# jzhou316/meta-gcn

Measured on AMD Instinct MI355X. Metric: edges/sec GCN fwd+bwd, 10M-edge synth graph F=128, at 1/2/4/8 MI355X, higher is better.
Workload: dtype f32; 1 GPU; config2: Erdos-Renyi N=1M, E=10M (+1M self-loops), F=128, 3-layer GCN (sm, add, bias, ReLU) fwd+bwd; nodes=1000000, edges=10000000, nnz=11000000, feat=128, layers=3, global_batch=1, parallelism=single

## Files before the change

meta-gcn_amd/csrc/fused.hip:

```cpp

#include <string>

#include "mgcn_internal.h"
#include "x6.h"

#ifndef MGCN_NT_AUX
#define MGCN_NT_AUX 2
#endif
#ifndef MGCN_NT_OUT
#define MGCN_NT_OUT 2
#endif

namespace mgcn {
namespace {

using namespace x6;

constexpr int kXwF = 128;
constexpr int kXwRows = 32;
constexpr int kXwWaves = 8;
constexpr int kXwThreads = 64 * kXwWaves;
constexpr int kXwImg = kXwRows * 256;
constexpr int kXwStageLd = kXwF + 8;
constexpr int kXwStage = kXwRows * kXwStageLd * 4;
// ... 292 lines not shown
        mcb = col[mb.beg + my];
        if (w != nullptr) mwb = w[mb.beg + my];
        if constexpr (MAXM) msb = slot_map[mb.beg + my];
      }
    }
    const int64_t ra = da - e0, rb = db - e0;
    const int na = ra <= 0 ? 0 : (ra < 32 ? (int)ra : 32);
    const int nb = rb <= 0 ? 0 : (rb < 32 ? (int)rb : 32);
    const int64_t remw = dm - e0;
    const int nbmax = remw < 32 ? (int)remw : 32;
    for (int k0 = 0; k0 < nbmax; k0 += U) {
      float4 xa[U], xb[U];
      float wa[U], wb[U];
      uint32_t ba[U], bb[U];
#pragma unroll
      for (int u = 0; u < U; ++u) {
        const int k = k0 + u;
        const int ca = bcast_g(mca, grp, k & 31);
        const int cb = bcast_g(mcb, grp, k & 31);
        wa[u] = bcast_g(mwa, grp, k & 31);
        wb[u] = bcast_g(mwb, grp, k & 31);
        const uint32_t oa = k < na ? (uint32_t)ca * ldx_b + 16u * gl : 0xfffffff0u;
        const uint32_t ob = k < nb ? (uint32_t)cb * ldx_b + 16u * gl : 0xfffffff0u;
        xa[u] = __builtin_bit_cast(float4, __builtin_amdgcn_raw_buffer_load_b128(rx, oa, 0, 0));
        xb[u] = __builtin_bit_cast(float4, __builtin_amdgcn_raw_buffer_load_b128(rx, ob, 0, 0));
        if constexpr (MAXM) {
          const int sa = bcast_g(msa, grp, k & 31);
          const int sb = bcast_g(msb, grp, k & 31);
          ba[u] = win[k < na ? (int64_t)sa * 4 + (gl >> 3) : 0];
          bb[u] = win[k < nb ? (int64_t)sb * 4 + (gl >> 3) : 0];
        }
      }
#pragma unroll
      for (int u = 0; u < U; ++u) {
        if constexpr (MAXM) {
          const uint32_t qa = ba[u] >> (4 * (gl & 7)), qb = bb[u] >> (4 * (gl & 7));
          xa[u].x = (qa & 1u) ? xa[u].x : 0.0f;
          xa[u].y = (qa & 2u) ? xa[u].y : 0.0f;
          xa[u].z = (qa & 4u) ? xa[u].z : 0.0f;
          xa[u].w = (qa & 8u) ? xa[u].w : 0.0f;
          xb[u].x = (qb & 1u) ? xb[u].x : 0.0f;
          xb[u].y = (qb & 2u) ? xb[u].y : 0.0f;
          xb[u].z = (qb & 4u) ? xb[u].z : 0.0f;
          xb[u].w = (qb & 8u) ? xb[u].w : 0.0f;
        }
        if (k0 + u < na) {
          aa[0] = __fadd_rn(aa[0], __fmul_rn(xa[u].x, wa[u]));
          aa[1] = __fadd_rn(aa[1], __fmul_rn(xa[u].y, wa[u]));
          aa[2] = __fadd_rn(aa[2], __fmul_rn(xa[u].z, wa[u]));
          aa[3] = __fadd_rn(aa[3], __fmul_rn(xa[u].w, wa[u]));
        }
        if (k0 + u < nb) {
          ab[0] = __fadd_rn(ab[0], __fmul_rn(xb[u].x, wb[u]));
          ab[1] = __fadd_rn(ab[1], __fmul_rn(xb[u].y, wb[u]));
          ab[2] = __fadd_rn(ab[2], __fmul_rn(xb[u].z, wb[u]));
          ab[3] = __fadd_rn(ab[3], __fmul_rn(xb[u].w, wb[u]));
        }
      }
    }
  }
}

struct RowSeq {
  int64_t base;
  int64_t step;
  int64_t n_rows;
  __device__ __forceinline__ int64_t row(int64_t k) const { return base + (k >> 1) * step + 16 * (k & 1); }
};

__device__ __forceinline__ int64_t my_chunks(int64_t n_chunks) {
  return blockIdx.x < n_chunks ? (n_chunks - 1 - blockIdx.x) / gridDim.x + 1 : 0;
}

#if MGCN_EXPERIMENT
constexpr int kTailMaxWg = 1024;
__device__ unsigned long long g_tail[2][kTailMaxWg][4];
#define XTAIL_ENTRY(k)                                           \
  if (threadIdx.x == 0 && blockIdx.x < kTailMaxWg) g_tail[k][blockIdx.x][0] = wall_clock64();
#define XTAIL_EXIT(k, chunks)                                                         \
  if ((threadIdx.x & 63) == 0 && blockIdx.x < kTailMaxWg) {                           \
    atomicMax(&g_tail[k][blockIdx.x][1], (unsigned long long)wall_clock64());         \
    if (threadIdx.x == 0) g_tail[k][blockIdx.x][2] = (unsigned long long)(chunks);    \
  }
#else
#define XTAIL_ENTRY(k)
#define XTAIL_EXIT(k, chunks)
#endif

__device__ __forceinline__ void store_row_terms(char *img_base, int lr, int gl, const float (&v)[4]) {
  uint32_t hi[2], mid[2], lo[2];
  split3_pair(f32x2{v[0], v[1]}, hi[0], mid[0], lo[0]);
  split3_pair(f32x2{v[2], v[3]}, hi[1], mid[1], lo[1]);
  char *img = img_base + img_off(lr, gl >> 1) + 8 * (gl & 1);
  *reinterpret_cast<uint2 *>(img) = make_uint2(hi[0], hi[1]);
  *reinterpret_cast<uint2 *>(img + kXwImg) = make_uint2(mid[0], mid[1]);
  *reinterpret_cast<uint2 *>(img + 2 * kXwImg) = make_uint2(lo[0], lo[1]);
}

__device__ __forceinline__ void mfma_rows(const char *img, const bf16x8 (&b)[3], int ks, int l16,
                                          int g4, f32x4_t (&acc)[2]) {
#pragma unroll
  for (int t = 0; t < 2; ++t) {
    const int off = img_off(16 * t + l16, 4 * ks + g4);
    const bf16x8 ah = *reinterpret_cast<const bf16x8 *>(img + off);
    const bf16x8 am = *reinterpret_cast<const bf16x8 *>(img + kXwImg + off);
    const bf16x8 al = *reinterpret_cast<const bf16x8 *>(img + 2 * kXwImg + off);
    acc[t] = mfma16_x6(ah, am, al, b[0], b[1], b[2], acc[t]);
  }
}

constexpr int kXfBuf = 3 * kXwImg;
constexpr int kXfStageOff = 2 * kXfBuf;
constexpr int kXfLds = kXfStageOff + 2 * kXfStage;
static_assert(2 * kXfLds <= 160 * 1024, "two forward workgroups per CU");

struct XwArgs {
  int64_t n_rows;
  const int64_t *rowptr;
  const int32_t *col;
  const float *w;
  const float *X;
  int64_t ldx;
  int64_t n_cols;
  const float *W;
  int64_t ldw;
  const float *bias;
  float *Y;
  int64_t ldy;
  uint32_t *relu_mask;
  float *Z;
  int64_t ldz;
  int mean;
  int relu;
  int32_t dyn_first;
  uint32_t *claim;
  int32_t *mail;
  const uint32_t *pk;
  uint32_t pk_bytes, pk_rbits, pk_head;
  uint32_t pk_base[64];
};

template <int U, bool PK = false, bool DYN = false>
__global__ __launch_bounds__(kXwThreads, 2 * kXwPerCU) void spmm_xw_fwd_kernel(const XwArgs a) {
  static_assert(!(DYN && PK), "the dynamic claim serves the dense forward");
  __shared__ __attribute__((aligned(16))) char lds[kXfLds];
  const int tid = threadIdx.x;
  const int lane = tid & 63;
  const int wave = __builtin_amdgcn_readfirstlane(tid >> 6);
  const int gl = lane & 31, grp = lane >> 5;
  const int l16 = lane & 15, g4 = lane >> 4;
  const int64_t n_chunks = (a.n_rows + kXwRows - 1) / kXwRows;
  const bool has_b = a.bias != nullptr;
  const auto rx = buf_rsrc(PK ? nullptr : a.X, PK ? 0u : (uint32_t)(a.n_cols * a.ldx * 4));
  const uint32_t ldx_b = (uint32_t)a.ldx * 4u;
  Pk128 pk{};
  u32x2 hh[PK ? U : 1];
  if constexpr (PK) {
    pk.r = buf_rsrc(a.pk, a.pk_bytes);
    pk.rbits = a.pk_rbits;
    pk.head = a.pk_head;
    pk.base = a.pk_base[lane];
  }

  const int ncol = 16 * wave + l16;
  bf16x8 wb[4][3];
  {
    const float *wp = a.W + (int64_t)(8 * g4) * a.ldw + ncol;
#pragma unroll
    for (int ks = 0; ks < 4; ++ks) {
// ... 481 lines not shown
  if (g_xw_dyn_rounds <= 0 || g_xw_unroll != 5 || workspace == nullptr ||
      reinterpret_cast<uintptr_t>(workspace) % 4 != 0 || workspace_bytes < xw_dyn_workspace_bytes() || rounds < g_xw_dyn_rounds + 8 ||
      n_chunks >= (int64_t(1) << 30))
    return false;
  a.dyn_first = (int32_t)((rounds - g_xw_dyn_rounds) * grid);
  a.claim = static_cast<uint32_t *>(workspace);
  a.mail = reinterpret_cast<int32_t *>(static_cast<char *>(workspace) + kXwDynMailOff);
  if (hipMemsetAsync(a.claim, 0, sizeof(uint32_t), s) != hipSuccess) {
    *rc = check_launch("hipMemsetAsync");
    return true;
  }
  hipLaunchKernelGGL((spmm_xw_fwd_kernel<5, false, true>), dim3((unsigned)grid), dim3(kXwThreads),
                     0, s, a);
  *rc = check_launch("spmm_xw_fwd_kernel");
  return true;
}

template <int U, bool DX, int EPI, bool MAXM, bool DW = true, bool PK = false>
int launch_xb(const XbArgs &a, int grid, hipStream_t s) {
  hipLaunchKernelGGL((spmm_xw_bwd_kernel<U, DX, EPI, MAXM, DW, PK>), dim3((unsigned)grid),
                     dim3(kXwThreads), 0, s, a);
  return check_launch("spmm_xw_bwd_kernel");
}

template <int U, bool PK = false>
int launch_xb_dx(const XbArgs &a, int epi, int grid, hipStream_t s) {
  if (epi == EPI_RELU_DIV) return launch_xb<U, true, EPI_RELU_DIV, false, false, PK>(a, grid, s);
  if (epi == EPI_RELU) return launch_xb<U, true, EPI_RELU, false, false, PK>(a, grid, s);
  return launch_xb<U, true, EPI_STORE, false, false, PK>(a, grid, s);
}

template <int U, bool MAXM>
int launch_xb_m(const XbArgs &a, int epi, int grid, hipStream_t s) {
  if (a.dX == nullptr) return launch_xb<U, false, EPI_STORE, MAXM>(a, grid, s);
  if (epi == EPI_RELU_DIV) return launch_xb<U, true, EPI_RELU_DIV, MAXM>(a, grid, s);
  if (epi == EPI_RELU) return launch_xb<U, true, EPI_RELU, MAXM>(a, grid, s);
  return launch_xb<U, true, EPI_STORE, MAXM>(a, grid, s);
}

template <int U>
int launch_xb_u(const XbArgs &a, int epi, int grid, hipStream_t s) {
  return a.win_mask != nullptr ? launch_xb_m<U, true>(a, epi, grid, s)
                               : launch_xb_m<U, false>(a, epi, grid, s);
}

constexpr int kBsDws = 2, kBsDwsH = 3, kBsDwsM = 4;
#ifndef MGCN_DS_MASK_RING
#define MGCN_DS_MASK_RING 1
#endif
constexpr int kBsImgSet = 3 * kXwImg;
constexpr int kDsXLd = kXwF + 4;
constexpr int kDsXOff = kBsImgSet;
constexpr int kDsMaskOff = kDsXOff + kXwRows * kDsXLd * 4;
constexpr int kDsDivOff = kDsMaskOff + kXwRows * 16;
constexpr int kDsRingBuf = kDsDivOff + kXwRows * 4;
constexpr int kDsWOff = 2 * kDsRingBuf;
constexpr int kDsCtrOff = kDsWOff + kXwF * kDsXLd * 4;
constexpr int kDsLds = kDsCtrOff + 64;
static_assert(kDsLds <= 160 * 1024, "one DWS workgroup per CU");
static_assert(16 * kXwF * 4 <= kDsWOff, "column-sum fold fits in the ring");
constexpr int kBsNG = 8, kBsNM = 8;
constexpr int kBsThreads = 64 * (kBsNG + kBsNM);

__device__ __forceinline__ int bs_lds_load(const int *p) {
  return __builtin_amdgcn_readfirstlane(
      __hip_atomic_load(p, __ATOMIC_RELAXED, __HIP_MEMORY_SCOPE_WORKGROUP));
}

__device__ __forceinline__ bool bs_wait_ge(const int *p, int target, int *abort_word,
                                           uint32_t limit) {
  for (uint32_t n = 0;; ++n) {
    if (bs_lds_load(p) >= target) break;
    if (bs_lds_load(abort_word) != 0) return false;
    if (n >= limit) {
      __hip_atomic_store(abort_word, 1, __ATOMIC_RELAXED, __HIP_MEMORY_SCOPE_WORKGROUP);
      return false;
    }
    __builtin_amdgcn_s_sleep(1);
  }
  asm volatile("" ::: "memory");
  return true;
}

__device__ __forceinline__ int bs_signal(int *p, int v, int lane) {
  asm volatile("s_waitcnt lgkmcnt(0)" ::: "memory");
  int old = 0;
  if (lane == 0) old = __hip_atomic_fetch_add(p, v, __ATOMIC_RELAXED, __HIP_MEMORY_SCOPE_WORKGROUP);
  return __builtin_amdgcn_readfirstlane(old);
}

__device__ __forceinline__ f32x4_t mfma16_x6_at(const bf16x8 (&w)[3], const bf16x8 &xh,
                                               const bf16x8 &xm, const bf16x8 &xl, f32x4_t c) {
  c = __builtin_amdgcn_mfma_f32_16x16x32_bf16(w[0], xl, c, 0, 0, 0);
  c = __builtin_amdgcn_mfma_f32_16x16x32_bf16(w[2], xh, c, 0, 0, 0);
  c = __builtin_amdgcn_mfma_f32_16x16x32_bf16(w[1], xm, c, 0, 0, 0);
  c = __builtin_amdgcn_mfma_f32_16x16x32_bf16(w[0], xm, c, 0, 0, 0);
  c = __builtin_amdgcn_mfma_f32_16x16x32_bf16(w[1], xh, c, 0, 0, 0);
  return __builtin_amdgcn_mfma_f32_16x16x32_bf16(w[0], xh, c, 0, 0, 0);
}

struct XbsArgs {
  XbArgs b;
  float *hcs_partial;
  int dbg;
  uint32_t spin;
  unsigned *err;
};

template <int U, int EPI, int MODE>
__global__ __launch_bounds__(kBsThreads) void spmm_xw_bwd_ws_kernel(const XbsArgs A) {
  constexpr bool HCS = MODE == kBsDwsH;
  constexpr bool MAXM = MODE == kBsDwsM;
  constexpr bool MRING = MGCN_DS_MASK_RING;
  constexpr int kRing = kDsRingBuf;
  constexpr int kDbgMask = MAXM ? ~0 : mgcn::kDbgMask;
  const XbArgs &a = A.b;
  __shared__ __attribute__((aligned(16))) char lds[kDsLds];
  const int tid = threadIdx.x;
  const int lane = tid & 63;
  const int wave = __builtin_amdgcn_readfirstlane(tid >> 6);
  const int gl = lane & 31, grp = lane >> 5;
  const int l16 = lane & 15, g4 = lane >> 4;
  int *ctr = reinterpret_cast<int *>(lds + kDsCtrOff);
  int *filled = ctr, *mdone = ctr + 2, *freed = ctr + 4, *abort_word = ctr + 8;
  if (tid < 16) ctr[tid] = 0;
#pragma unroll
  for (int j = 0; j < 4; ++j) {
    const int e = tid + kBsThreads * j;
    const float4 v = *reinterpret_cast<const float4 *>(a.W + (int64_t)(e >> 5) * a.ldw + 4 * (e & 31));
    *reinterpret_cast<float4 *>(lds + kDsWOff + 4 * ((e >> 5) * kDsXLd + 4 * (e & 31))) = v;
  }
  __syncthreads();

  const int64_t n_chunks = (a.n_rows + kXwRows - 1) / kXwRows;
  const int64_t n_my = my_chunks(n_chunks);
  auto chunk_of = [&](int64_t i) { return (int64_t)blockIdx.x + i * gridDim.x; };
  XTAIL_ENTRY(1);
  auto rows_in = [&](int64_t c) -> uint32_t {
    const int64_t r = a.n_rows - c * kXwRows;
    return (uint32_t)(r <= 0 ? 0 : r >= kXwRows ? kXwRows : r);
  };

  float cs[4] = {0.0f, 0.0f, 0.0f, 0.0f};
  float hc[4] = {0.0f, 0.0f, 0.0f, 0.0f};
  f32x16 accw[2];
#pragma unroll
  for (int s = 0; s < 2; ++s)
#pragma unroll
    for (int r = 0; r < 16; ++r) accw[s][r] = 0.0f;

  if (wave < kBsNG) {
    const int64_t n_quads = 8 * n_my;
    auto row_of = [&](int64_t k, int second) -> int64_t {
      const int64_t q = wave + kBsNG * k;
      return chunk_of(q >> 3) * kXwRows + 4 * (q & 7) + 2 * second + grp;
    };
    const auto rdy = buf_rsrc(a.dY, (uint32_t)(a.n_cols * a.lddy * 4));
    const uint32_t ldy_b = (uint32_t)a.lddy * 4u;
    RowMeta cur[2] = {}, nxt[2] = {};
#pragma unroll
    for (int j = 0; j < 2; ++j) {
      meta_rowptr(a.rowptr, row_of(0, j), row_of(0, j) < a.n_rows && wave < n_quads, cur[j]);
      if constexpr (MAXM)
        meta_first_m(a.col, a.w, a.slot_map, gl, cur[j]);
      else
        meta_first(a.col, a.w, gl, cur[j]);
      meta_rowptr(a.rowptr, row_of(1, j), row_of(1, j) < a.n_rows && wave + kBsNG < n_quads,
                  nxt[j]);
    }
    int64_t k = 0;
    for (int64_t q = wave; q < n_quads; q += kBsNG, ++k) {
      RowMeta nn[2];
#pragma unroll
      for (int j = 0; j < 2; ++j) {
        if constexpr (MAXM)
          meta_first_m(a.col, a.w, a.slot_map, gl, nxt[j]);
        else
          meta_first(a.col, a.w, gl, nxt[j]);
        const int64_t r2 = row_of(k + 2, j);
        meta_rowptr(a.rowptr, r2, r2 < a.n_rows && q + 2 * kBsNG < n_quads, nn[j]);
      }
      const int64_t i = q >> 3;
      const int64_t c = chunk_of(i);
      const int64_t r0 = c * kXwRows;
      const int lr0 = 4 * (int)(q & 7) + grp;
      u32x4 zv[2] = {};
      if (!(A.dbg & kDbgMask & 4)) {
        const auto rz = buf_rsrc(a.X + r0 * a.ldx, rows_in(c) * (uint32_t)a.ldx * 4u);
#pragma unroll
        for (int j = 0; j < 2; ++j)
          zv[j] = __builtin_amdgcn_raw_buffer_load_b128(
              rz, 4 * (int)((lr0 + 2 * j) * a.ldx + 4 * gl), 0, MGCN_NT_AUX);
      }
      uint32_t mv[2] = {0u, 0u};
      if constexpr (MRING && EPI != EPI_STORE) {
        const auto rm = buf_rsrc(a.relu_mask + r0 * 4, rows_in(c) * 16u);
#pragma unroll
        for (int j = 0; j < 2; ++j)
          if (gl < 4) mv[j] = __builtin_amdgcn_raw_buffer_load_b32(rm, 4 * ((lr0 + 2 * j) * 4 + gl), 0, 0);
        if constexpr (EPI == EPI_RELU_DIV) {
          const auto rd = buf_rsrc(a.row_div + r0, rows_in(c) * 4u);
#pragma unroll
          for (int j = 0; j < 2; ++j)
            if (gl == 4) mv[j] = __builtin_amdgcn_raw_buffer_load_b32(rd, 4 * (lr0 + 2 * j), 0, 0);
        }
      }
      u32x4 yv[2] = {};
      if constexpr (HCS) {
        const auto ry = buf_rsrc(a.dY + r0 * a.lddy, rows_in(c) * (uint32_t)a.lddy * 4u);
#pragma unroll
        for (int j = 0; j < 2; ++j)
          yv[j] = __builtin_amdgcn_raw_buffer_load_b128(
              ry, 4 * (int)((lr0 + 2 * j) * a.lddy + 4 * gl), 0, 0);
      }
      float acc[2][4];
      gather_row2_meta<U, MAXM>(rdy, ldy_b, a.col, a.w, cur[0], cur[1], gl, grp, acc[0], acc[1],
                                a.win_mask, a.slot_map);
      if constexpr (HCS) {
#pragma unroll
        for (int j = 0; j < 2; ++j) {
          const float4 y = __builtin_bit_cast(float4, yv[j]);
          hc[0] = __fadd_rn(hc[0], y.x);
          hc[1] = __fadd_rn(hc[1], y.y);
          hc[2] = __fadd_rn(hc[2], y.z);
          hc[3] = __fadd_rn(hc[3], y.w);
        }
      }
#pragma unroll
      for (int j = 0; j < 2; ++j) {
        const int64_t row = r0 + lr0 + 2 * j;
        if (a.row_scale != nullptr && row < a.n_rows) {
          const float sc = a.row_scale[row];
#pragma unroll
          for (int t = 0; t < 4; ++t) acc[j][t] = __fmul_rn(acc[j][t], sc);
        }
      }
      const int b = (int)(i & 1);
      const int gen = (int)(i >> 1);
      if (!bs_wait_ge(freed + b, gen, abort_word, A.spin)) break;
      char *buf = lds + b * kRing;
#pragma unroll
      for (int j = 0; j < 2; ++j) {
        store_row_terms(buf, lr0 + 2 * j, gl, acc[j]);
        *reinterpret_cast<u32x4 *>(buf + kDsXOff + 4 * ((lr0 + 2 * j) * kDsXLd + 4 * gl)) = zv[j];
        if constexpr (MRING && EPI != EPI_STORE) {
          if (gl < 4)
            *reinterpret_cast<uint32_t *>(buf + kDsMaskOff + 4 * ((lr0 + 2 * j) * 4 + gl)) = mv[j];
          if (EPI == EPI_RELU_DIV && gl == 4)
            *reinterpret_cast<uint32_t *>(buf + kDsDivOff + 4 * (lr0 + 2 * j)) = mv[j];
        }
      }
      bs_signal(filled + b, 4, lane);
#pragma unroll
      for (int j = 0; j < 2; ++j) {
        cur[j] = nxt[j];
        nxt[j] = nn[j];
      }
    }
  } else {
    const int m = wave - kBsNG;
    const int ti = m >> 1, tj0 = 2 * (m & 1);
    auto read8 = [&](const char *base, const int (&o)[2]) {
      const v4i16 x0 = __builtin_amdgcn_ds_read_tr16_b64_v4i16((lds_v4i16_t *)(base + o[0]));
      const v4i16 x1 = __builtin_amdgcn_ds_read_tr16_b64_v4i16((lds_v4i16_t *)(base + o[1]));
      const short y[8] = {x0[0], x0[1], x0[2], x0[3], x1[0], x1[1], x1[2], x1[3]};
      return __builtin_bit_cast(bf16x8, y);
    };
    const int bit = 4 * m + g4;
    for (int64_t i = 0; i < n_my; ++i) {
      int lane_o = lane;
      asm volatile("" : "+v"(lane_o));
      const int l16 = lane_o & 15, g4 = lane_o >> 4, h = lane_o >> 5;
      int offb[2][2];
      {
        const int q = (lane_o >> 2) & 3, p4 = lane_o & 3;
#pragma unroll
        for (int s2 = 0; s2 < 2; ++s2)
#pragma unroll
          for (int r = 0; r < 2; ++r)
            offb[s2][r] = img_off(8 * h + q + 4 * r, 4 * (tj0 + s2) + 2 * (g4 & 1) + (p4 >> 1)) +
                          8 * (p4 & 1);
      }
      const int b = (int)(i & 1);
      const int gen = (int)(i >> 1);
      const int64_t c = chunk_of(i);
      const int64_t r0 = c * kXwRows;
      const uint32_t rv = rows_in(c);
      u32x4 mk[2] = {};
      float dv[2] = {1.0f, 1.0f};
      if constexpr (EPI != EPI_STORE && !MRING) {
        const auto rm = buf_rsrc(a.relu_mask + r0 * 4, rv * 16u);
#pragma unroll
        for (int rt = 0; rt < 2; ++rt)
          mk[rt] = __builtin_amdgcn_raw_buffer_load_b128(rm, 16 * (16 * rt + l16), 0, 0);
        if constexpr (EPI == EPI_RELU_DIV) {
          const auto rd = buf_rsrc(a.row_div + r0, rv * 4u);
#pragma unroll
          for (int rt = 0; rt < 2; ++rt)
            dv[rt] = __uint_as_float(__builtin_amdgcn_raw_buffer_load_b32(rd, 4 * (16 * rt + l16), 0, 0));
        }
      }
      if (!bs_wait_ge(filled + b, kXwRows * (gen + 1), abort_word, A.spin)) break;
      uint32_t mbits[2] = {0u, 0u};
      if constexpr (EPI != EPI_STORE && MRING) {
#pragma unroll
        for (int rt = 0; rt < 2; ++rt) {
          const u32x4 w4 = *reinterpret_cast<const u32x4 *>(lds + b * kRing + kDsMaskOff + 16 * (16 * rt + l16));
#pragma unroll
          for (int r = 0; r < 4; ++r) mbits[rt] |= ((w4[r] >> bit) & 1u) << r;
          if constexpr (EPI == EPI_RELU_DIV)
            dv[rt] = *reinterpret_cast<const float *>(lds + b * kRing + kDsDivOff + 4 * (16 * rt + l16));
        }
      }
      if constexpr (EPI == EPI_RELU_DIV) {
#pragma unroll
        for (int rt = 0; rt < 2; ++rt)
          if ((uint32_t)(16 * rt + l16) >= rv) dv[rt] = 1.0f;
      }
      const char *buf = lds + b * kRing;
      {
          if (!(A.dbg & kDbgMask & 1)) {
          const float *xr = reinterpret_cast<const float *>(buf + kDsXOff) + 32 * ti + (lane_o & 31);
#pragma unroll
          for (int ks = 0; ks < 2; ++ks) {
            float xv[8];
#pragma unroll
            for (int j = 0; j < 8; ++j) xv[j] = xr[(16 * ks + 8 * h + j) * kDsXLd];
            bf16x8 fa[3];
            split3_bf16(xv, fa[0], fa[1], fa[2]);
#pragma unroll
            for (int s2 = 0; s2 < 2; ++s2) {
              bf16x8 fb[3];
#pragma unroll
              for (int t = 0; t < 3; ++t) fb[t] = read8(buf + ks * 16 * 256 + t * kXwImg, offb[s2]);
              accw[s2] = mfma_x6(fa[0], fa[1], fa[2], fb[0], fb[1], fb[2], accw[s2]);
            }
          }
        }
        }
      const auto rx = buf_rsrc(a.dX + r0 * a.lddx, rv * (uint32_t)a.lddx * 4u);
      f32x4_t acc2[2];
#pragma unroll
      for (int rt = 0; rt < 2; ++rt)
#pragma unroll
        for (int r = 0; r < 4; ++r) acc2[rt][r] = 0.0f;
      const float *wq = reinterpret_cast<const float *>(lds + kDsWOff) + (16 * m + l16) * kDsXLd + 8 * g4;
      float4 wn0{}, wn1{};
      if (!(A.dbg & kDbgMask & 8)) {
        wn0 = *reinterpret_cast<const float4 *>(wq);
        wn1 = *reinterpret_cast<const float4 *>(wq + 4);
      }
      if (a.dX != nullptr) {
#pragma unroll
      for (int ks = 0; ks < 4; ++ks) {
        bf16x8 wk[3];
        {
          const float v8[8] = {wn0.x, wn0.y, wn0.z, wn0.w, wn1.x, wn1.y, wn1.z, wn1.w};
              if (ks + 1 < 4 && !(A.dbg & kDbgMask & 8)) {
            wn0 = *reinterpret_cast<const float4 *>(wq + 32 * (ks + 1));
            wn1 = *reinterpret_cast<const float4 *>(wq + 32 * (ks + 1) + 4);
          }
              split3_bf16(v8, wk[0], wk[1], wk[2]);
        }
#pragma unroll
        for (int rt = 0; rt < 2; ++rt) {
          const int off = img_off(16 * rt + l16, 4 * ks + g4);
          const bf16x8 xh = *reinterpret_cast<const bf16x8 *>(buf + off);
          const bf16x8 xm = *reinterpret_cast<const bf16x8 *>(buf + kXwImg + off);
          const bf16x8 xl = *reinterpret_cast<const bf16x8 *>(buf + 2 * kXwImg + off);
          acc2[rt] = mfma16_x6_at(wk, xh, xm, xl, acc2[rt]);
        }
      }
#pragma unroll
      for (int rt = 0; rt < 2; ++rt) {
        const int row = 16 * rt + l16;
        float v[4];
#pragma unroll
        for (int r = 0; r < 4; ++r) {
          v[r] = acc2[rt][r];
          if constexpr (EPI != EPI_STORE) {
            const uint32_t on = MRING ? (mbits[rt] >> r) & 1u : (mk[rt][r] >> bit) & 1u;
            v[r] = on ? v[r] : 0.0f;
            cs[r] = __fadd_rn(cs[r], v[r]);
            if constexpr (EPI == EPI_RELU_DIV) v[r] = __fdiv_rn(v[r], dv[rt]);
          }
        }
        __builtin_amdgcn_raw_buffer_store_b128(
            __builtin_bit_cast(u32x4, make_float4(v[0], v[1], v[2], v[3])), rx,
            4 * (int)(row * a.lddx + 16 * m + 4 * g4), 0, MGCN_NT_OUT);
      }
      }
      const int old = bs_signal(mdone + b, 1, lane);
      if (old == kBsNM * gen + kBsNM - 1) bs_signal(freed + b, 1, lane);
    }
  }
  __syncthreads();
  if (wave == 0 && bs_lds_load(abort_word) != 0) report_device_error(A.err, kDevErrDws);
  if (wave >= kBsNG) {
    const int m = wave - kBsNG;
    {
      const int h = lane >> 5, lc = lane & 31;
      const int ti = m >> 1, tj0 = 2 * (m & 1);
      float *slab = a.dw_partial + (int64_t)blockIdx.x * kXwF * kXwF;
#pragma unroll
      for (int s2 = 0; s2 < 2; ++s2)
#pragma unroll
        for (int r = 0; r < 16; ++r) {
          const int row = 32 * ti + (r & 3) + 8 * (r >> 2) + 4 * h;
          slab[row * kXwF + 32 * (tj0 + s2) + lc] = accw[s2][r];
        }
    }
    if constexpr (EPI != EPI_STORE) {
      float *red = reinterpret_cast<float *>(lds);
      *reinterpret_cast<float4 *>(red + l16 * kXwF + 16 * m + 4 * g4) =
          make_float4(cs[0], cs[1], cs[2], cs[3]);
    }
  }
  if constexpr (HCS) {
    float *red2 = reinterpret_cast<float *>(lds) + 16 * kXwF;
    if (wave < kBsNG)
      *reinterpret_cast<float4 *>(red2 + (2 * wave + grp) * kXwF + 4 * gl) =
          make_float4(hc[0], hc[1], hc[2], hc[3]);
  }
  if (EPI != EPI_STORE || HCS) {
    __syncthreads();
    if constexpr (EPI != EPI_STORE) {
      if (tid < kXwF) {
        const float *red = reinterpret_cast<const float *>(lds);
        float s = 0.0f;
#pragma unroll
        for (int l = 0; l < 16; ++l) s = __fadd_rn(s, red[l * kXwF + tid]);
        a.colsum_partial[(int64_t)blockIdx.x * kXwF + tid] = s;
      }
    }
    if (HCS && tid >= kXwF && tid < 2 * kXwF) {
      const int f = tid - kXwF;
      const float *red2 = reinterpret_cast<const float *>(lds) + 16 * kXwF;
      float s = 0.0f;
#pragma unroll
      for (int l = 0; l < 16; ++l) s = __fadd_rn(s, red2[l * kXwF + f]);
      A.hcs_partial[(int64_t)blockIdx.x * kXwF + f] = s;
    }
  }
  XTAIL_EXIT(1, n_my);
}

int g_xw_ws_full = 1;
int g_xw_ws_max = 1;

int bs_grid() {
  int dev = 0, cus = 256;
  if (hipGetDevice(&dev) != hipSuccess ||
      hipDeviceGetAttribute(&cus, hipDeviceAttributeMultiprocessorCount, dev) != hipSuccess)
    cus = 256;
  return cus;
}

template <int U, int MODE>
int launch_bs_u(const XbsArgs &a, int epi, int grid, hipStream_t s) {
  if (epi == EPI_RELU_DIV)
    hipLaunchKernelGGL((spmm_xw_bwd_ws_kernel<U, EPI_RELU_DIV, MODE>), dim3(grid), dim3(kBsThreads),
                       0, s, a);
  else if (epi == EPI_RELU)
    hipLaunchKernelGGL((spmm_xw_bwd_ws_kernel<U, EPI_RELU, MODE>), dim3(grid), dim3(kBsThreads), 0,
                       s, a);
  else
    hipLaunchKernelGGL((spmm_xw_bwd_ws_kernel<U, EPI_STORE, MODE>), dim3(grid), dim3(kBsThreads), 0,
                       s, a);
  return check_launch("spmm_xw_bwd_ws_kernel");
}

int g_bs_dbg = 0;

int g_bs_full_unroll = 5;

template <int MODE>
int launch_bs(const XbsArgs &a, int epi, int grid, hipStream_t s) {
  if constexpr (MODE == kBsDwsM) {
    return launch_bs_u<3, MODE>(a, epi, grid, s);
  } else {
    return g_bs_full_unroll == 4 ? launch_bs_u<4, MODE>(a, epi, grid, s)
         : g_bs_full_unroll == 5 ? launch_bs_u<5, MODE>(a, epi, grid, s)
                                 : launch_bs_u<6, MODE>(a, epi, grid, s);
  }
}

int bs_prepare(XbsArgs &sa) {
  sa.dbg = MGCN_EXPERIMENT ? g_bs_dbg : 0;
  sa.spin = g_spin_limit;
  sa.err = device_error_word();
  return sa.err == nullptr ? MGCN_EHIP : MGCN_OK;
}

}

int xw_set_ws(const char *name, int value) {
  const std::string n(name);
  auto flag = [&](int &g) {
    if (value < 0 || value > 1) {
      set_error("%s must be 0 or 1", name);
      return (int)MGCN_EINVAL;
    }
    g = value;
    return (int)MGCN_OK;
  };
  auto unroll = [&](int &g, std::initializer_list<int> ok) {
    for (int v : ok)
      if (v == value) {
        g = value;
        return (int)MGCN_OK;
      }
    set_error("%s: unsupported value %d", name, value);
    return (int)MGCN_EINVAL;
  };
  if (n == "xw_pk_unroll" || n == "xw_pk_bwd_unroll") {
    if (!MGCN_EXPERIMENT) {
      set_error("%s: experiment builds only (make exp -> libmgcn_exp.so)", name);
      return MGCN_EINVAL;
    }
    return n == "xw_pk_unroll" ? unroll(g_xw_pk_unroll, {3, 4, 5, 6})
                               : unroll(g_xw_pk_bwd_unroll, {2, 3, 4});
  }
  if (n == "xw_ws_max") return flag(g_xw_ws_max);
  if (n == "xw_ws_full") return flag(g_xw_ws_full);
  if (n == "xw_ws_dbg") {
    if (!MGCN_EXPERIMENT) {
      set_error("xw_ws_dbg: experiment builds only (make exp -> libmgcn_exp.so)");
      return MGCN_EINVAL;
    }
    g_bs_dbg = value;
    return MGCN_OK;
  }
  return unroll(g_bs_full_unroll, {4, 5, 6});
}

int xw_set_dyn_rounds(int value) {
  if (value < 0 || value > 64) {
    set_error("xw_dyn_rounds must be in 0 .. 64 (0: no dynamic claim)");
    return MGCN_EINVAL;
  }
  g_xw_dyn_rounds = value;
  return MGCN_OK;
}

int xw_set_unroll(int value) {
  if (value != 4 && value != 5 && value != 6 && value != 8) {
    set_error("spmm_xw_unroll must be 4, 5, 6 or 8 (5 / 6: the forward only)");
    return MGCN_EINVAL;
  }
  g_xw_unroll = value;
  return MGCN_OK;
}

}

using namespace mgcn;

extern "C" int mgcn_spmm_xw_supported(int32_t F_in, int32_t F_out, int reduce) {
  return F_in == F_out && (F_in == kXwF || F_in == 256) && gemm_precision_is_x6() &&
         (reduce == MGCN_REDUCE_SUM || reduce == MGCN_REDUCE_MEAN);
}

extern "C" int mgcn_spmm_xw_bwd_full_supported(int32_t F_in, int32_t F_out) {
  return F_in == kXwF && F_out == kXwF && gemm_precision_is_x6();
}

extern "C" size_t mgcn_spmm_xw_fwd_workspace_bytes(int32_t F_in, int32_t F_out) {
  if (F_in == kXwF && F_out == kXwF) return xw_dyn_workspace_bytes();
  return F_in == 256 && F_out == 256 ? xw_wide_workspace_bytes(false) : 0;
}

extern "C" int mgcn_spmm_xw_fwd(int64_t n_rows, int64_t n_cols, int32_t F_in, int32_t F_out,
                                const int64_t *rowptr, const int32_t *col, const float *w,
                                const float *X, int64_t ldx, const float *W, int64_t ldw,
                                const float *bias, float *Y, int64_t ldy, int reduce, int relu,
                                uint32_t *relu_mask, float *Z, int64_t ldz, void *workspace,
                                size_t workspace_bytes, void *stream) {
  clear_error();
  if (int rc = take_device_error()) return rc;
  MGCN_REQUIRE(n_rows >= 0, "mgcn_spmm_xw_fwd: negative size");
  MGCN_REQUIRE(mgcn_spmm_xw_supported(F_in, F_out, reduce),
               "mgcn_spmm_xw_fwd: unsupported F_in=%d F_out=%d reduce=%d (needs 128 x 128 or "
               "256 x 256, sum/mean, bf16x6)",
               F_in, F_out, reduce);
  MGCN_REQUIRE(relu_mask == nullptr || relu, "mgcn_spmm_xw_fwd: relu_mask needs relu");
  if (n_rows == 0) return MGCN_OK;
  MGCN_REQUIRE(rowptr && X && W && Y, "mgcn_spmm_xw_fwd: null array");
  MGCN_REQUIRE(ldx >= F_in && ldx % 4 == 0 && reinterpret_cast<uintptr_t>(X) % 16 == 0,
               "mgcn_spmm_xw_fwd: X must have 16-byte aligned rows");
  MGCN_REQUIRE(ldw >= F_out && ldy >= F_out, "mgcn_spmm_xw_fwd: leading dimension too small");
  if (F_in == 256) {
    MGCN_REQUIRE(n_cols > 0 && (uint64_t)16 * (uint64_t)(ldy > ldz ? ldy : ldz) * 4u < (1ull << 31),
                 "mgcn_spmm_xw_fwd: leading dimension too large");
    MGCN_REQUIRE(relu_mask == nullptr || reinterpret_cast<uintptr_t>(relu_mask) % 16 == 0,
                 "mgcn_spmm_xw_fwd: relu_mask not 16-byte aligned");
    MGCN_REQUIRE(Z == nullptr || (ldz >= F_in && ldz % 4 == 0 && reinterpret_cast<uintptr_t>(Z) % 16 == 0),
                 "mgcn_spmm_xw_fwd: Z must have 16-byte aligned rows (ldz >= F_in)");
    MGCN_REQUIRE(ldy % 4 == 0 && reinterpret_cast<uintptr_t>(Y) % 16 == 0,
                 "mgcn_spmm_xw_fwd: Y must have 16-byte aligned rows at F = 256");
    const size_t need = mgcn_spmm_xw_fwd_workspace_bytes(F_in, F_out);
    if (workspace == nullptr || workspace_bytes < need) {
      set_error("mgcn_spmm_xw_fwd: workspace %zu < %zu", workspace_bytes, need);
      return MGCN_EWORKSPACE;
    }
    return xw_wide_fwd(n_rows, rowptr, col, w, X, ldx, W, ldw, bias, Y, ldy,
                       reduce == MGCN_REDUCE_MEAN, relu != 0, relu_mask, Z, ldz, workspace,
// ... 130 lines not shown
  a.dY = dY;
  a.lddy = lddy;
  a.n_cols = n_cols;
  a.X = X;
  a.ldx = ldx;
  a.W = W;
  a.ldw = ldw;
  a.dX = dX;
  a.lddx = lddx;
  a.relu_mask = relu_mask;
  a.row_div = row_div;
  a.win_mask = win_mask;
  a.slot_map = slot_map;
  a.dw_partial = static_cast<float *>(workspace);
  a.colsum_partial = reinterpret_cast<float *>(static_cast<char *>(workspace) +
                                               align_up((size_t)xw_grid() * kXwF * kXwF * 4, 256));
  int rc;
  if (dx_only) {
    rc = g_xw_unroll == 8 ? launch_xb_dx<8>(a, epi, grid, s) : launch_xb_dx<4>(a, epi, grid, s);
    if (rc || epi == EPI_STORE) return rc;
    return launch_fold(a.colsum_partial, grid, kXwF, kXwF, colsum, kXwF, accumulate, s);
  }
  float *hcs_partial = nullptr;
  if ((g_xw_ws_full || dy_colsum) && (win_mask == nullptr || (g_xw_ws_max && dX != nullptr))) {
    XbsArgs sa{};
    sa.b = a;
    if (int rc2 = bs_prepare(sa)) return rc2;
    grid = bs_grid() < n_chunks ? bs_grid() : (int)n_chunks;
    if (dy_colsum) hcs_partial = a.dw_partial + (size_t)grid * kXwF * kXwF;
    sa.hcs_partial = hcs_partial;
    rc = hcs_partial ? launch_bs<kBsDwsH>(sa, epi, grid, s)
         : win_mask  ? launch_bs<kBsDwsM>(sa, epi, grid, s)
                     : launch_bs<kBsDws>(sa, epi, grid, s);
  } else {
    rc = g_xw_unroll == 8 ? launch_xb_u<8>(a, epi, grid, s) : launch_xb_u<4>(a, epi, grid, s);
  }
  if (rc) return rc;
  rc = launch_split_reduce(a.dw_partial, grid, (int64_t)kXwF * kXwF, kXwF, dW, lddw, accumulate, s);
  if (rc == MGCN_OK && hcs_partial) rc = launch_colsum_fold(hcs_partial, grid, kXwF, dy_colsum, s);
  if (rc || epi == EPI_STORE) return rc;
  return launch_colsum_fold(a.colsum_partial, grid, kXwF, colsum, s);
}
}

extern "C" int mgcn_spmm_xw_bwd(int64_t n_rows, int64_t n_cols, int32_t F_in, int32_t F_out,
                                const int64_t *rowptr_t, const int32_t *col_t, const float *w_t,
                                const float *row_scale, const float *dY, int64_t lddy,
                                const float *X, int64_t ldx, const float *W, int64_t ldw,
                                float *dW, int64_t lddw, int accumulate, float *dX, int64_t lddx,
                                const uint32_t *relu_mask, const float *row_div, float *colsum,
                                const uint32_t *win_mask, const int32_t *slot_map,
                                void *workspace, size_t workspace_bytes, void *stream) {
  clear_error();
  return xw_bwd_impl(n_rows, n_cols, F_in, F_out, rowptr_t, col_t, w_t, row_scale, dY, lddy, X,
                     ldx, W, ldw, dW, lddw, accumulate, dX, lddx, relu_mask, row_div, colsum,
                     win_mask, slot_map, nullptr, workspace, workspace_bytes, stream);
}

extern "C" int mgcn_spmm_xw_bwd_hcs(int64_t n_rows, int64_t n_cols, const int64_t *rowptr_t,
                                    const int32_t *col_t, const float *w_t,
                                    const float *row_scale, const float *dY, int64_t lddy,
                                    const float *X, int64_t ldx, const float *W, int64_t ldw,
                                    float *dW, int64_t lddw, int accumulate, float *dX,
                                    int64_t lddx, const uint32_t *relu_mask,
                                    const float *row_div, float *colsum, float *dy_colsum,
                                    void *workspace, size_t workspace_bytes, void *stream) {
  clear_error();
  MGCN_REQUIRE(n_rows == n_cols, "mgcn_spmm_xw_bwd_hcs: needs n_rows == n_cols (%lld, %lld): "
               "every dY row a row of the view", (long long)n_rows, (long long)n_cols);
  MGCN_REQUIRE(X != nullptr && dW != nullptr && dX != nullptr && dy_colsum != nullptr,
               "mgcn_spmm_xw_bwd_hcs: X, dW, dX and dy_colsum are required");
  return xw_bwd_impl(n_rows, n_cols, kXwF, kXwF, rowptr_t, col_t, w_t, row_scale, dY, lddy, X,
                     ldx, W, ldw, dW, lddw, accumulate, dX, lddx, relu_mask, row_div, colsum,
                     nullptr, nullptr, dy_colsum, workspace, workspace_bytes, stream);
}

#if MGCN_EXPERIMENT
extern "C" int mgcn_debug_xw_tail(unsigned long long *host) {
  MGCN_HIP_TRY(hipDeviceSynchronize());
  if (host != nullptr)
    MGCN_HIP_TRY(hipMemcpyFromSymbol(host, HIP_SYMBOL(g_tail), sizeof(g_tail)));
  static const unsigned long long zero[2][kTailMaxWg][4] = {};
  MGCN_HIP_TRY(hipMemcpyToSymbol(HIP_SYMBOL(g_tail), zero, sizeof(zero)));
  return MGCN_OK;
}
#endif

#ifdef MGCN_XW_PROFILE
extern "C" int mgcn_debug_xw_prof(unsigned long long *host) {
  MGCN_HIP_TRY(hipDeviceSynchronize());
  MGCN_HIP_TRY(hipMemcpyFromSymbol(host, HIP_SYMBOL(g_xprof), sizeof(g_xprof)));
  return MGCN_OK;
}
#endif

namespace {
int check_packed(const mgcn_packed_table *t, int32_t F, const char *who) {
  MGCN_REQUIRE(t != nullptr && t->words != nullptr, "%s: null packed table", who);
  MGCN_REQUIRE(t->F == F, "%s: packed table of F = %d for a layer of F = %d", who, t->F, F);
  MGCN_REQUIRE(t->n_seg >= 1 && t->n_seg <= 64, "%s: n_seg %d outside 1 .. 64", who, t->n_seg);
  MGCN_REQUIRE(t->row_bits >= 0 && t->row_bits + 6 <= 31 && t->seg_rows >= 1 &&
                   (int64_t)t->seg_rows <= ((int64_t)1 << t->row_bits),
               "%s: seg_rows %d does not fit row_bits %d", who, t->seg_rows, t->row_bits);
  MGCN_REQUIRE((uint64_t)t->seg_rows * (2 * (F / 32) + F) * 4u + 16u < (1ull << 31),
               "%s: seg_rows %d too large for the 2-GiB in-segment offsets", who, t->seg_rows);
  MGCN_REQUIRE(t->n_words >= 0, "%s: negative n_words", who);
  if (F == kXwF) {
    MGCN_REQUIRE((uint64_t)t->n_words * 4u <= 0x7ffffff0ull,
                 "%s: an F = 128 packed table spans at most 2 GiB - 16 B (got %lld words)", who,
                 (long long)t->n_words);
    for (int s = 0; s < t->n_seg; ++s)
      MGCN_REQUIRE(t->seg_base[s] >= 0 && t->seg_base[s] <= t->n_words,
                   "%s: segment %d at word %lld outside the table's %lld words", who, s,
                   (long long)t->seg_base[s], (long long)t->n_words);
  }
  return MGCN_OK;
}

template <class Args>
void fill_pk128(Args &a, const mgcn_packed_table *t) {
  a.pk = t->words;
  a.pk_bytes = (uint32_t)(t->n_words * 4);
  a.pk_rbits = (uint32_t)t->row_bits;
  a.pk_head = (uint32_t)t->seg_rows * 8u;
  for (int s = 0; s < 64; ++s) a.pk_base[s] = s < t->n_seg ? (uint32_t)t->seg_base[s] : 0u;
}
}

extern "C" int mgcn_spmm_xw_fwd_packed(int64_t n_rows, int32_t F_in, int32_t F_out,
                                       const int64_t *rowptr, const int32_t *col, const float *w,
                                       const mgcn_packed_table *X, const float *W, int64_t ldw,
                                       const float *bias, float *Y, int64_t ldy, int reduce,
                                       int relu, uint32_t *relu_mask, float *Z, int64_t ldz,
                                       void *workspace, size_t workspace_bytes, void *stream) {
  clear_error();
  if (int rc = take_device_error()) return rc;
  MGCN_REQUIRE(n_rows >= 0, "mgcn_spmm_xw_fwd_packed: negative size");
  MGCN_REQUIRE(mgcn_spmm_xw_supported(F_in, F_out, reduce),
               "mgcn_spmm_xw_fwd_packed: 128 x 128 or 256 x 256, sum / mean, bf16x6 only");
  MGCN_REQUIRE(relu_mask == nullptr || relu, "mgcn_spmm_xw_fwd_packed: relu_mask needs relu");
  if (n_rows == 0) return MGCN_OK;
  if (int rc = check_packed(X, F_in, "mgcn_spmm_xw_fwd_packed")) return rc;
  MGCN_REQUIRE(rowptr && W && Y, "mgcn_spmm_xw_fwd_packed: null array");
  if (F_in == kXwF) {
    MGCN_REQUIRE(ldw >= F_out && ldy >= F_out && (uint64_t)kXwRows * (uint64_t)ldy * 4u < (1ull << 31),
                 "mgcn_spmm_xw_fwd_packed: bad ldw / ldy");
    MGCN_REQUIRE(bias == nullptr || reinterpret_cast<uintptr_t>(bias) % 4 == 0,
                 "mgcn_spmm_xw_fwd_packed: bias not 4-byte aligned");
    MGCN_REQUIRE(relu_mask == nullptr || reinterpret_cast<uintptr_t>(relu_mask) % 16 == 0,
                 "mgcn_spmm_xw_fwd_packed: relu_mask not 16-byte aligned");
    MGCN_REQUIRE(Z == nullptr || (ldz >= F_in && ldz % 4 == 0 && reinterpret_cast<uintptr_t>(Z) % 16 == 0 &&
                                  (uint64_t)kXwRows * (uint64_t)ldz * 4u < (1ull << 31)),
                 "mgcn_spmm_xw_fwd_packed: Z must have 16-byte aligned rows (ldz >= F_in)");
    XwArgs a{};
    a.n_rows = n_rows;
    a.rowptr = rowptr;
    a.col = col;
    a.w = w;
    a.W = W;
    a.ldw = ldw;
    a.bias = bias;
    a.Y = Y;
    a.ldy = ldy;
    a.relu_mask = relu_mask;
    a.Z = Z;
    a.ldz = ldz;
// ... 109 lines not shown
```

meta-gcn_amd/csrc/spmm.hip:

```cpp

#include <hipcub/hipcub.hpp>

#include "heavy.h"
#include "mgcn_internal.h"

namespace mgcn {
namespace {

constexpr int kWaves = 4;
constexpr int kBlock = 64 * kWaves;

template <int G>
__device__ __forceinline__ int bcast_i(int v, int group_base, int k) {
  if constexpr (G == 64) {
    return __builtin_amdgcn_readlane(v, k);
  } else {
    return __shfl(v, group_base + k, 64);
  }
}
template <int G>
__device__ __forceinline__ float bcast_f(float v, int group_base, int k) {
  return __int_as_float(bcast_i<G>(__float_as_int(v), group_base, k));
}

// ... 581 lines not shown
    }
  }
  if (n_heavy > n_giant)
    return bwd ? launch_heavy_v<BWD_SUM>(a, vec, false, stream)
               : launch_heavy_v<FWD_SUM>(a, vec, false, stream);
  return MGCN_OK;
}

int heavy_rows_join(hipStream_t stream) {
  SideStream *side = nullptr;
  if (int rc = side_stream(&side)) return rc;
  MGCN_HIP_TRY(hipStreamWaitEvent(stream, side->join, 0));
  return MGCN_OK;
}

}

using namespace mgcn;

#ifdef MGCN_HEAVY_PROFILE
extern "C" int mgcn_debug_heavy_prof(unsigned long long *host) {
  MGCN_HIP_TRY(hipDeviceSynchronize());
  MGCN_HIP_TRY(hipMemcpyFromSymbol(host, HIP_SYMBOL(g_hprof), sizeof(g_hprof)));
  return MGCN_OK;
}
#endif

extern "C" int mgcn_set_option(const char *name, int value) {
  clear_error();
  MGCN_REQUIRE(name != nullptr, "mgcn_set_option: null name");
  const std::string n(name);
  if (n == "spmm_vec") {
    MGCN_REQUIRE(value == 0 || value == 1 || value == 2 || value == 4, "spmm_vec must be 0,1,2,4");
    g_force_vec = value;
    return MGCN_OK;
  }
  if (n == "spmm_unroll") {
    MGCN_REQUIRE(value == 4 || value == 6 || value == 8 || value == 16,
                 "spmm_unroll must be 4, 6, 8 or 16");
    g_unroll = value;
    g_unroll_set = true;
    return MGCN_OK;
  }
  if (n == "heavy_lds_kb") {
    MGCN_REQUIRE(value >= 16 && value <= 160, "heavy_lds_kb must be in [16, 160]");
    g_heavy_lds = value * 1024;
    return MGCN_OK;
  }
  if (n == "heavy_block") {
    MGCN_REQUIRE(value == 256 || value == 512 || value == 1024, "heavy_block must be 256, 512 or 1024");
    g_heavy_block = value;
    return MGCN_OK;
  }
  if (n == "heavy_mid_q1") {
    MGCN_REQUIRE(value == 0 || value == 1, "heavy_mid_q1 must be 0 or 1");
    g_heavy_mid_q1 = value;
    return MGCN_OK;
  }
  if (n == "heavy_mid_lds_kb") {
    MGCN_REQUIRE(value >= 16 && value <= 160, "heavy_mid_lds_kb must be in [16, 160]");
    g_heavy_mid_lds = value * 1024;
    return MGCN_OK;
  }
  if (n == "heavy_giant_thr") {
    MGCN_REQUIRE(value >= 0, "heavy_giant_thr must be >= 0");
    g_giant_thr = value;
    return MGCN_OK;
  }
  if (n == "gemm_tn_variant") {
    MGCN_REQUIRE(value >= 0 && value <= 2, "gemm_tn_variant must be 0, 1 or 2");
    return gemm_set_tn_variant(value);
  }
  if (n == "gemm_tn_staged") {
    MGCN_REQUIRE(value == 0 || value == 1, "gemm_tn_staged must be 0 or 1");
    return gemm_set_tn_staged(value);
  }
  if (n == "gemm_precision") {
    MGCN_REQUIRE(value == 0 || value == 1, "gemm_precision must be 0 (f32) or 1 (bf16x6)");
    return gemm_set_precision(value);
  }
  if (n == "spmm_xw_unroll") return xw_set_unroll(value);
  if (n == "xw_dyn_rounds") return xw_set_dyn_rounds(value);
  if (n == "xw_ws_dbg" || n == "xw_ws_full" || n == "xw_ws_max" || n == "xw_ws_full_unroll" ||
      n == "xw_pk_unroll" || n == "xw_pk_bwd_unroll")
    return xw_set_ws(name, value);
  if (n == "wide_pair" || n == "wide_ws" || n == "wide_dbg" || n == "wide_mfma") return wide_set_option(name, value);
  if (n == "residual_blocks") {
    MGCN_REQUIRE(value >= 64 && value <= 65536, "residual_blocks must be in [64, 65536]");
    g_rl_cap = value;
    return MGCN_OK;
  }
  if (n == "residual_fused_mask") {
    MGCN_REQUIRE(value == 0 || value == 1, "residual_fused_mask must be 0 or 1");
    g_fused_mask = value;
    return MGCN_OK;
  }
  if (n == "heavy_side_fence") {
    MGCN_REQUIRE(value == 0 || value == 1, "heavy_side_fence must be 0 or 1");
    g_side_fence = value;
    return MGCN_OK;
  }
  if (n == "ws_spin_limit") {
    if (!MGCN_EXPERIMENT) {
      set_error("ws_spin_limit: experiment builds only (make exp -> libmgcn_exp.so)");
      return MGCN_EINVAL;
    }
    MGCN_REQUIRE(value >= 1, "ws_spin_limit must be >= 1");
    g_spin_limit = (uint32_t)value;
    return MGCN_OK;
  }
  if (n == "heavy_side_stream") {
    MGCN_REQUIRE(value == 0 || value == 1, "heavy_side_stream must be 0 or 1");
    g_heavy_side = value;
    return MGCN_OK;
  }
  set_error("mgcn_set_option: unknown option '%s'", name);
  return MGCN_EINVAL;
}

static int choose_vec(int32_t F, const void *p0, int64_t ld0, const void *p1, int64_t ld1) {
  int v = pick_vec(F, p0, ld0, p1, ld1);
  if (g_force_vec != 0 && g_force_vec < v) v = g_force_vec;
  return v;
}

extern "C" int mgcn_spmm_fwd(int64_t n_rows, int32_t F, const int64_t *rowptr, const int32_t *col,
                             const int32_t *eid, const float *w, const float *H, int64_t ldh,
                             float *Y, int64_t ldy, int reduce, const float *bias, int relu,
                             int32_t *argmax, uint32_t *win_mask, uint32_t *relu_mask,
                             const int32_t *order, int64_t n_heavy, int64_t n_giant,
                             void *stream) {
  clear_error();
  MGCN_REQUIRE(n_rows >= 0 && F >= 0, "mgcn_spmm_fwd: negative size");
  MGCN_REQUIRE(relu_mask == nullptr || (relu && F <= 128),
               "mgcn_spmm_fwd: relu_mask needs relu and F <= 128");
  MGCN_REQUIRE(reduce == MGCN_REDUCE_SUM || reduce == MGCN_REDUCE_MEAN || reduce == MGCN_REDUCE_MAX,
               "mgcn_spmm_fwd: bad reduce %d", reduce);
  if (n_rows == 0 || F == 0) return MGCN_OK;
  MGCN_REQUIRE(rowptr && H && Y, "mgcn_spmm_fwd: null array");
  MGCN_REQUIRE(ldh >= F && ldy >= F, "mgcn_spmm_fwd: leading dimension < F");
  MGCN_REQUIRE(reduce != MGCN_REDUCE_MAX || argmax != nullptr || win_mask != nullptr,
               "mgcn_spmm_fwd: MAX needs argmax and/or win_mask (+ eid)");
  SpmmArgs a{};
  a.n_rows = n_rows;
  a.F = F;
  a.rowptr = rowptr;
  a.col = col;
  a.eid = eid;
  a.w = w;
  a.X = H;
  a.ldx = ldh;
  a.Y = Y;
  a.ldy = ldy;
  a.bias = bias;
  a.argmax_out = argmax;
  a.win_mask_out = reduce == MGCN_REDUCE_MAX ? win_mask : nullptr;
  a.relu_mask = relu_mask;
  MGCN_REQUIRE(order == nullptr || (0 <= n_giant && n_giant <= n_heavy && n_heavy <= n_rows),
               "spmm: need 0 <= n_giant <= n_heavy <= n_rows");
  a.order = order;
  a.n_heavy = n_heavy;
  a.n_giant = n_giant;
  a.mean = reduce == MGCN_REDUCE_MEAN;
  a.relu = relu != 0;
  int vec = choose_vec(F, H, ldh, Y, ldy);
  if (reduce == MGCN_REDUCE_MAX && argmax != nullptr &&
// ... 173 lines not shown
```

Before: 6.181 billion edges/s.

## Hand out gather quads in the backward warp-specialized kernel via an LDS ticket counter

After: 6.236 billion edges/s (median of 6 runs). Within noise of the previous version (+0.9%).

```diff
diff --git a/meta-gcn_amd/csrc/fused.hip b/meta-gcn_amd/csrc/fused.hip
--- a/meta-gcn_amd/csrc/fused.hip
+++ b/meta-gcn_amd/csrc/fused.hip
@@ -398,9 +398,27 @@
     atomicMax(&g_tail[k][blockIdx.x][1], (unsigned long long)wall_clock64());         \
     if (threadIdx.x == 0) g_tail[k][blockIdx.x][2] = (unsigned long long)(chunks);    \
   }
+__device__ unsigned long long g_dws_wait[kTailMaxWg][4];
+#define XWAIT_DECL uint32_t xw_wait = 0, xw_t0 = (uint32_t)wall_clock64(), xw_w0 = 0
+#define XWAIT_BEGIN xw_w0 = (uint32_t)wall_clock64()
+#define XWAIT_BEGIN_DRAINED                            \
+  asm volatile("s_waitcnt vmcnt(0)" ::: "memory"); \
+  XWAIT_BEGIN
+#define XWAIT_END xw_wait += (uint32_t)wall_clock64() - xw_w0
+#define XWAIT_STORE(k)                                                                \
+  if ((threadIdx.x & 63) == 0 && blockIdx.x < kTailMaxWg) {                           \
+    atomicAdd(&g_dws_wait[blockIdx.x][2 * (k)], (unsigned long long)xw_wait);         \
+    atomicAdd(&g_dws_wait[blockIdx.x][2 * (k) + 1],                                   \
+              (unsigned long long)((uint32_t)wall_clock64() - xw_t0));                \
+  }
 #else
 #define XTAIL_ENTRY(k)
 #define XTAIL_EXIT(k, chunks)
+#define XWAIT_DECL
+#define XWAIT_BEGIN
+#define XWAIT_BEGIN_DRAINED
+#define XWAIT_END
+#define XWAIT_STORE(k)
 #endif
 
 __device__ __forceinline__ void store_row_terms(char *img_base, int lr, int gl, const float (&v)[4]) {
@@ -1048,6 +1066,12 @@
   return true;
 }
 
+__device__ __forceinline__ int bs_draw(int *p, int lane) {
+  int t = 0;
+  if (lane == 0) t = __hip_atomic_fetch_add(p, 1, __ATOMIC_RELAXED, __HIP_MEMORY_SCOPE_WORKGROUP);
+  return __builtin_amdgcn_readfirstlane(t);
+}
+
 __device__ __forceinline__ int bs_signal(int *p, int v, int lane) {
   asm volatile("s_waitcnt lgkmcnt(0)" ::: "memory");
   int old = 0;
@@ -1073,8 +1097,9 @@
   unsigned *err;
 };
 
-template <int U, int EPI, int MODE>
+template <int U, int EPI, int MODE, bool CLAIM = false>
 __global__ __launch_bounds__(kBsThreads) void spmm_xw_bwd_ws_kernel(const XbsArgs A) {
+  static_assert(!CLAIM || MODE == kBsDws, "hcs_partial folds per gather wave in quad order");
   constexpr bool HCS = MODE == kBsDwsH;
   constexpr bool MAXM = MODE == kBsDwsM;
   constexpr bool MRING = MGCN_DS_MASK_RING;
@@ -1089,7 +1114,8 @@
   const int l16 = lane & 15, g4 = lane >> 4;
   int *ctr = reinterpret_cast<int *>(lds + kDsCtrOff);
   int *filled = ctr, *mdone = ctr + 2, *freed = ctr + 4, *abort_word = ctr + 8;
-  if (tid < 16) ctr[tid] = 0;
+  int *ticket = ctr + 10;
+  if (tid < 16) ctr[tid] = CLAIM && tid == 10 ? kBsNG : 0;
 #pragma unroll
   for (int j = 0; j < 4; ++j) {
     const int e = tid + kBsThreads * j;
@@ -1121,6 +1147,10 @@
       const int64_t q = wave + kBsNG * k;
       return chunk_of(q >> 3) * kXwRows + 4 * (q & 7) + 2 * second + grp;
     };
+    auto row_of_quad = [&](int64_t q, int second) -> int64_t {
+      return chunk_of(q >> 3) * kXwRows + 4 * (q & 7) + 2 * second + grp;
+    };
+    XWAIT_DECL;
     const auto rdy = buf_rsrc(a.dY, (uint32_t)(a.n_cols * a.lddy * 4));
     const uint32_t ldy_b = (uint32_t)a.lddy * 4u;
     RowMeta cur[2] = {}, nxt[2] = {};
@@ -1131,20 +1161,28 @@
         meta_first_m(a.col, a.w, a.slot_map, gl, cur[j]);
       else
         meta_first(a.col, a.w, gl, cur[j]);
-      meta_rowptr(a.rowptr, row_of(1, j), row_of(1, j) < a.n_rows && wave + kBsNG < n_quads,
-                  nxt[j]);
+      if constexpr (!CLAIM)
+        meta_rowptr(a.rowptr, row_of(1, j), row_of(1, j) < a.n_rows && wave + kBsNG < n_quads,
+                    nxt[j]);
     }
     int64_t k = 0;
-    for (int64_t q = wave; q < n_quads; q += kBsNG, ++k) {
+    for (int64_t q = wave; q < n_quads; ++k) {
       RowMeta nn[2];
+      int64_t q_nxt = 0;
+      if constexpr (CLAIM) q_nxt = bs_draw(ticket, lane);
 #pragma unroll
       for (int j = 0; j < 2; ++j) {
-        if constexpr (MAXM)
-          meta_first_m(a.col, a.w, a.slot_map, gl, nxt[j]);
-        else
-          meta_first(a.col, a.w, gl, nxt[j]);
-        const int64_t r2 = row_of(k + 2, j);
-        meta_rowptr(a.rowptr, r2, r2 < a.n_rows && q + 2 * kBsNG < n_quads, nn[j]);
+        if constexpr (CLAIM) {
+          const int64_t r1 = row_of_quad(q_nxt, j);
+          meta_rowptr(a.rowptr, r1, r1 < a.n_rows && q_nxt < n_quads, nxt[j]);
+        } else {
+          if constexpr (MAXM)
+            meta_first_m(a.col, a.w, a.slot_map, gl, nxt[j]);
+          else
+            meta_first(a.col, a.w, gl, nxt[j]);
+          const int64_t r2 = row_of(k + 2, j);
+          meta_rowptr(a.rowptr, r2, r2 < a.n_rows && q + 2 * kBsNG < n_quads, nn[j]);
+        }
       }
       const int64_t i = q >> 3;
       const int64_t c = chunk_of(i);
@@ -1182,6 +1220,10 @@
       float acc[2][4];
       gather_row2_meta<U, MAXM>(rdy, ldy_b, a.col, a.w, cur[0], cur[1], gl, grp, acc[0], acc[1],
                                 a.win_mask, a.slot_map);
+      if constexpr (CLAIM) {
+#pragma unroll
+        for (int j = 0; j < 2; ++j) meta_first(a.col, a.w, gl, nxt[j]);
+      }
       if constexpr (HCS) {
 #pragma unroll
         for (int j = 0; j < 2; ++j) {
@@ -1203,7 +1245,9 @@
       }
       const int b = (int)(i & 1);
       const int gen = (int)(i >> 1);
+      XWAIT_BEGIN_DRAINED;
       if (!bs_wait_ge(freed + b, gen, abort_word, A.spin)) break;
+      XWAIT_END;
       char *buf = lds + b * kRing;
 #pragma unroll
       for (int j = 0; j < 2; ++j) {
@@ -1220,9 +1264,15 @@
 #pragma unroll
       for (int j = 0; j < 2; ++j) {
         cur[j] = nxt[j];
-        nxt[j] = nn[j];
-      }
-    }
+        if constexpr (!CLAIM) nxt[j] = nn[j];
+      }
+      if constexpr (CLAIM) {
+        q = q_nxt;
+      } else {
+        q += kBsNG;
+      }
+    }
+    XWAIT_STORE(0);
   } else {
     const int m = wave - kBsNG;
     const int ti = m >> 1, tj0 = 2 * (m & 1);
@@ -1233,6 +1283,7 @@
       return __builtin_bit_cast(bf16x8, y);
     };
     const int bit = 4 * m + g4;
+    XWAIT_DECL;
     for (int64_t i = 0; i < n_my; ++i) {
       int lane_o = lane;
       asm volatile("" : "+v"(lane_o));
@@ -1266,7 +1317,9 @@
             dv[rt] = __uint_as_float(__builtin_amdgcn_raw_buffer_load_b32(rd, 4 * (16 * rt + l16), 0, 0));
         }
       }
+      XWAIT_BEGIN;
       if (!bs_wait_ge(filled + b, kXwRows * (gen + 1), abort_word, A.spin)) break;
+      XWAIT_END;
       uint32_t mbits[2] = {0u, 0u};
       if constexpr (EPI != EPI_STORE && MRING) {
 #pragma unroll
@@ -1359,6 +1412,7 @@
       const int old = bs_signal(mdone + b, 1, lane);
       if (old == kBsNM * gen + kBsNM - 1) bs_signal(freed + b, 1, lane);
     }
+    XWAIT_STORE(1);
   }
   __syncthreads();
   if (wave == 0 && bs_lds_load(abort_word) != 0) report_device_error(A.err, kDevErrDws);
@@ -1422,29 +1476,33 @@
   return cus;
 }
 
-template <int U, int MODE>
+template <int U, int MODE, bool CLAIM = false>
 int launch_bs_u(const XbsArgs &a, int epi, int grid, hipStream_t s) {
   if (epi == EPI_RELU_DIV)
-    hipLaunchKernelGGL((spmm_xw_bwd_ws_kernel<U, EPI_RELU_DIV, MODE>), dim3(grid), dim3(kBsThreads),
-                       0, s, a);
+    hipLaunchKernelGGL((spmm_xw_bwd_ws_kernel<U, EPI_RELU_DIV, MODE, CLAIM>), dim3(grid),
+                       dim3(kBsThreads), 0, s, a);
   else if (epi == EPI_RELU)
-    hipLaunchKernelGGL((spmm_xw_bwd_ws_kernel<U, EPI_RELU, MODE>), dim3(grid), dim3(kBsThreads), 0,
-                       s, a);
+    hipLaunchKernelGGL((spmm_xw_bwd_ws_kernel<U, EPI_RELU, MODE, CLAIM>), dim3(grid),
+                       dim3(kBsThreads), 0, s, a);
   else
-    hipLaunchKernelGGL((spmm_xw_bwd_ws_kernel<U, EPI_STORE, MODE>), dim3(grid), dim3(kBsThreads), 0,
-                       s, a);
+    hipLaunchKernelGGL((spmm_xw_bwd_ws_kernel<U, EPI_STORE, MODE, CLAIM>), dim3(grid),
+                       dim3(kBsThreads), 0, s, a);
   return check_launch("spmm_xw_bwd_ws_kernel");
 }
 
 int g_bs_dbg = 0;
 
 int g_bs_full_unroll = 5;
+
+int g_xw_ws_claim = 1;
 
 template <int MODE>
 int launch_bs(const XbsArgs &a, int epi, int grid, hipStream_t s) {
   if constexpr (MODE == kBsDwsM) {
     return launch_bs_u<3, MODE>(a, epi, grid, s);
   } else {
+    if constexpr (MODE == kBsDws)
+      if (g_xw_ws_claim && g_bs_full_unroll == 5) return launch_bs_u<5, MODE, true>(a, epi, grid, s);
     return g_bs_full_unroll == 4 ? launch_bs_u<4, MODE>(a, epi, grid, s)
          : g_bs_full_unroll == 5 ? launch_bs_u<5, MODE>(a, epi, grid, s)
                                  : launch_bs_u<6, MODE>(a, epi, grid, s);
@@ -1488,6 +1546,7 @@
                                : unroll(g_xw_pk_bwd_unroll, {2, 3, 4});
   }
   if (n == "xw_ws_max") return flag(g_xw_ws_max);
+  if (n == "xw_ws_claim") return flag(g_xw_ws_claim);
   if (n == "xw_ws_full") return flag(g_xw_ws_full);
   if (n == "xw_ws_dbg") {
     if (!MGCN_EXPERIMENT) {
@@ -1784,6 +1843,17 @@
     MGCN_HIP_TRY(hipMemcpyFromSymbol(host, HIP_SYMBOL(g_tail), sizeof(g_tail)));
   static const unsigned long long zero[2][kTailMaxWg][4] = {};
   MGCN_HIP_TRY(hipMemcpyToSymbol(HIP_SYMBOL(g_tail), zero, sizeof(zero)));
+  return MGCN_OK;
+}
+#endif
+
+#if MGCN_EXPERIMENT
+extern "C" int mgcn_debug_dws_wait(unsigned long long *host) {
+  MGCN_HIP_TRY(hipDeviceSynchronize());
+  if (host != nullptr)
+    MGCN_HIP_TRY(hipMemcpyFromSymbol(host, HIP_SYMBOL(g_dws_wait), sizeof(g_dws_wait)));
+  static const unsigned long long zero[kTailMaxWg][4] = {};
+  MGCN_HIP_TRY(hipMemcpyToSymbol(HIP_SYMBOL(g_dws_wait), zero, sizeof(zero)));
   return MGCN_OK;
 }
 #endif
diff --git a/meta-gcn_amd/csrc/spmm.hip b/meta-gcn_amd/csrc/spmm.hip
--- a/meta-gcn_amd/csrc/spmm.hip
+++ b/meta-gcn_amd/csrc/spmm.hip
@@ -687,6 +687,7 @@
   if (n == "spmm_xw_unroll") return xw_set_unroll(value);
   if (n == "xw_dyn_rounds") return xw_set_dyn_rounds(value);
   if (n == "xw_ws_dbg" || n == "xw_ws_full" || n == "xw_ws_max" || n == "xw_ws_full_unroll" ||
+      n == "xw_ws_claim" ||
       n == "xw_pk_unroll" || n == "xw_pk_bwd_unroll")
     return xw_set_ws(name, value);
   if (n == "wide_pair" || n == "wide_ws" || n == "wide_dbg" || n == "wide_mfma") return wide_set_option(name, value);
```
